# strawberrylady99/mythril

Measured on AMD Instinct MI355X. Metric: candidate assignments evaluated/sec (node) + time-to-first-model vs z3, higher is better.
Workload: dtype u32

## Files before the change

### mythril_amd/csrc/jit_asm.cpp

```cpp
#include <algorithm>
#include <array>
#include <cstdio>
#include <cstring>
#include <functional>
#include <map>
#include <set>
#include <sstream>
#include <string>
#include <vector>

#include "jit.hpp"

namespace mg {

namespace {

struct AsmFail {
  std::string why;
};
[[noreturn]] void fail(const std::string& w) { throw AsmFail{w}; }

inline uint32_t Lw(uint32_t w) { return (w + 31) / 32; }
inline uint32_t topmask(uint32_t w) { return (w & 31) ? ((1u << (w & 31)) - 1u) : 0xFFFFFFFFu; }
inline uint32_t gsalt(uint32_t c, uint32_t j) { return c * 0x9E3779B9u + j * 0x85EBCA6Bu + 0x27D4EB2Fu; }
// ... 31 lines not shown
  snprintf(b, sizeof b, "0x%x", x);
  return b;
}
bool inl(uint32_t x) {
  const int32_t s = (int32_t)x;
  return s >= -16 && s <= 64;
}
std::string imm(uint32_t x) { return inl(x) ? std::to_string((int32_t)x) : hexs(x); }
std::string V(uint32_t r) { return "v" + std::to_string(r); }
std::string S(uint32_t r) { return "s" + std::to_string(r); }
std::string SP(uint32_t r) { return "s[" + std::to_string(r) + ":" + std::to_string(r + 1) + "]"; }
std::string VP(uint32_t r) { return "v[" + std::to_string(r) + ":" + std::to_string(r + 1) + "]"; }

constexpr int kV0 = 12;
constexpr int kS0 = 44, kS1 = 100;

class Emitter {
 public:
  std::ostringstream o;
  int64_t pos = 0;
  std::map<int, int64_t> vw;
  int nlab = 0;
  std::vector<int> vref = std::vector<int>(256, 0);
  std::vector<uint32_t> vgen = std::vector<uint32_t>(256, 0);
  uint32_t gen_ctr = 0;
  static bool check_on() {
    static const bool on = [] {
      const char* g = getenv("MYTHGPU_JIT_ASM_CHECK");
      return g && g[0] == '1';
    }();
// ... 738 lines not shown
        E.valu("v_add3_u32 " + VL(vj) + ", " + VL(vj) + ", " + VL(ve) + ", " + (inl(base) ? imm(base) : "s41"), {41});
        E.valu("v_lshlrev_b32_e32 " + VL(vj) + ", 2, " + VL(vj));
        drop(vi);
        drop(ve);
        pend.push_back({vt, vj});
        if (pend.size() >= stage_batch()) flush();
      }
    }
    flush();
    E.ctl("s_waitcnt lgkmcnt(0)");
    E.ctl("s_barrier");
  }

  Emitter& e() { return E; }

  int cond = 0;
  static constexpr int kCondPairs = 8;
  void sreserve() {
    while (E.sfree() < kCondPairs && E.on_spressure && E.on_spressure()) {
    }
  }
  struct CondScope {
    Gen& g;
    explicit CondScope(Gen& g_) : g(g_) {
      if (!g.cond) g.sreserve();
      g.cond++;
    }
    ~CondScope() { g.cond--; }
  };
  std::map<uint32_t, Limb> litcache;
// ... 395 lines not shown
      const uint32_t e = cnt == 1 ? first : miss;
      const std::string op = cnt == 1 ? "v_cmp_eq_u32" : "v_cmp_ne_u32";
      if (inl(e)) {
        E.valu(op + "_e64 " + SP(m.s) + ", " + imm(e) + ", " + VL(idx), {}, {m.s, m.s + 1});
      } else {
        E.valu(op + "_e32 vcc, " + hexs(e) + ", " + VL(idx), {}, {kVCC, kVCC + 1});
        E.salu("s_mov_b64 " + SP(m.s) + ", vcc", {m.s, m.s + 1});
      }
      mcache_put(ck, m);
      return true;
    }
    uint32_t bits = 0;
    for (uint32_t e = 0; e < n; e++)
      if (S[e]) bits |= 1u << e;
    const Limb t = fresh();
    E.salu("s_mov_b32 s41, " + hexs(bits), {41});
    E.valu("v_bfe_u32 " + VL(t) + ", s41, " + VL(idx) + ", 1", {41});
    E.valu("v_cmp_ne_u32_e64 " + SP(m.s) + ", 0, " + VL(t), {}, {m.s, m.s + 1});
    drop(t);
    mcache_put(ck, m);
    return true;
  }
  bool dict_eq(const std::vector<std::pair<Limb, Limb>>& prs, Mask& m) {
    if (no_dict_eq() || dlimb.empty()) return false;
    bool haveA = false, haveB = false;
    DLimb A, B;
    std::vector<std::pair<uint32_t, uint32_t>> lits;
    std::vector<std::pair<uint32_t, uint32_t>> regs;
    auto same_src = [](const DLimb& x, const DLimb& y) {
      return x.off == y.off && x.n == y.n && x.Lc == y.Lc && x.idx == y.idx && x.idx.g == y.idx.g;
    };
    for (const auto& pr : prs) {
// ... 912 lines not shown
    const Limb d = into ? *into : fresh(), t = fresh();
    const uint32_t salt = gsalt(c, j);
    if (no_kfold()) {
      E.valu("v_xor_b32_e32 " + VL(d) + ", " + imm(salt) + ", v4");
      E.valu("v_xor_b32_sdwa " + VL(d) + ", " + VL(d) + ", " + VL(d) +
             " dst_sel:DWORD dst_unused:UNUSED_PAD src0_sel:DWORD src1_sel:WORD_1");
    } else {
      E.valu("v_xor_b32_e32 " + VL(d) + ", " + imm(salt ^ (salt >> 16)) + ", v4");
    }
    E.valu("v_mul_u32_u24_e32 " + VL(d) + ", 0x9e3779, " + VL(d));
    E.valu("v_lshrrev_b32_e32 " + VL(t) + ", 15, " + VL(d));
    E.valu("v_xad_u32 " + VL(d) + ", " + VL(t) + ", " + VL(d) + ", v5");
    drop(t);
    return d;
  }
  void gwsel(uint32_t c, int s) {
    E.salu("s_xor_b32 " + S(s) + ", s36, " + hexs(gsalt(c, 0xFFFEu)), {s});
    E.salu("s_mul_i32 " + S(s) + ", " + S(s) + ", 0x9e3779b1", {s});
    E.salu("s_add_u32 " + S(s) + ", " + S(s) + ", s37", {s});
  }
  std::vector<Limb> uniform_limbs(uint32_t c, uint32_t Lc, uint32_t bits, const std::vector<Limb>* tgt = nullptr) {
    const uint32_t n = std::min(Lc, (bits + 31) / 32);
    if (tgt) {
      std::vector<Limb> r(*tgt);
      for (uint32_t j = 0; j < n; j++) {
        if (j < 2) {
          grnd(c, j, &r[j]);
        } else {
          const uint32_t s = (7u * j + 3u) % 31u + 1u;
          E.valu("v_alignbit_b32 " + VL(r[j]) + ", " + VL(r[j - 1]) + ", " + VL(r[j - 2]) + ", " + std::to_string(s));
// ... 48 lines not shown
  }
  std::vector<Limb> add_lit(const uint32_t* lo, uint32_t Lc, const std::vector<Limb>& off, uint32_t k) {
    std::vector<Limb> a(k), b(k);
    for (uint32_t j = 0; j < k; j++) {
      a[j] = Lit(lo[j]);
      b[j] = j < off.size() ? off[j] : Lit(0);
    }
    std::vector<Limb> r = add_chain(a, b, k, false);
    r.resize(Lc);
    for (uint32_t j = k; j < Lc; j++) r[j] = Lit(lo[j]);
    return r;
  }
  Limb mulhi_lit(const Limb& x, uint32_t c) {
    if (x.lit()) return Lit((uint32_t)(((uint64_t)x.v * c) >> 32));
    const Limb d = fresh();
    if (inl(c)) {
      E.valu("v_mul_hi_u32 " + VL(d) + ", " + VL(x) + ", " + imm(c));
    } else {
      E.salu("s_mov_b32 s41, " + hexs(c), {41});
      E.valu("v_mul_hi_u32 " + VL(d) + ", " + VL(x) + ", s41", {41});
    }
    return d;
  }

  std::vector<Limb> dict(uint32_t off, uint32_t n, uint32_t w, const Limb& idx, const std::vector<Limb>* tgt = nullptr,
                         uint32_t upto = 64) {
    const uint32_t Lc = Lw(w), Lu = std::min(Lc, upto);
    std::vector<Limb> r(Lc, Lit(0));
    auto dst = [&](uint32_t j) { return tgt ? (*tgt)[j] : fresh(); };
    if (w <= 32 && n && (uint64_t)n * w <= 32) {
      uint32_t pack = 0;
      const uint32_t m = w == 32 ? 0xFFFFFFFFu : ((1u << w) - 1u);
      for (uint32_t e2 = 0; e2 < n; e2++) pack |= (G[off + e2] & m) << (e2 * w);
      const Limb sh = fresh(), d = dst(0);
      E.valu("v_mul_u32_u24_e32 " + VL(sh) + ", " + imm(w) + ", " + VL(idx));
      E.salu("s_mov_b32 s41, " + hexs(pack), {41});
      E.valu("v_bfe_u32 " + VL(d) + ", s41, " + VL(sh) + ", " + std::to_string(w), {41});
      drop(sh);
      r[0] = d;
      return r;
    }
    if (n <= 4 && !lds_base.count(off)) {
      std::vector<Mask> ms;
      for (uint32_t e2 = 0; e2 + 1 < n; e2++) {
        Mask m;
        m.k = 2;
        m.s = E.salloc();
        E.valu("v_cmp_ne_u32_e64 " + SP(m.s) + ", " + std::to_string(e2) + ", " + VL(idx), {}, {m.s, m.s + 1});
        ms.push_back(m);
      }
      std::map<std::vector<uint32_t>, Limb> memo;
      std::function<Limb(uint32_t, uint32_t)> chain = [&](uint32_t j, uint32_t e) -> Limb {
// ... 168 lines not shown
    E.valu("v_lshrrev_b32_e32 " + VL(e2) + ", 16, " + VL(e2));
    return e2;
  }

  void put(const std::vector<Limb>& out, std::vector<Limb>& r) {
    for (size_t j = 0; j < out.size(); j++) {
      const Limb x = j < r.size() ? r[j] : Lit(0);
      if (x == out[j]) continue;
      E.valu("v_mov_b32_e32 " + VL(out[j]) + ", " + src(x));
      if (j < r.size()) drop(r[j]);
    }
    for (size_t j = out.size(); j < r.size(); j++) drop(r[j]);
    r.clear();
  }

  void delta(const std::vector<Limb>& out, uint32_t c, uint32_t pdelta, int ws, const Limb* hknown) {
    CondScope cs_(*this);
    const std::string skip = E.newlab();
    E.salu("s_and_b32 s40, " + S(ws) + ", 0xffff", {40});
    E.salu("s_cmp_lt_u32 s40, " + imm(pdelta));
    E.ctl("s_cbranch_scc0 " + skip);
    Limb h = hknown ? *hknown : grnd(c, 0xFFFFu);
    if (hknown) E.retain(h);
    const Limb mag = fresh(), neg = fresh();
    Mask sb;
    sb.k = 2;
    sb.s = E.salloc();
    E.valu("v_and_b32_e32 " + VL(mag) + ", 1, " + VL(h));
    E.valu("v_add_u32_e32 " + VL(mag) + ", 1, " + VL(mag));
    E.valu("v_bfe_u32 " + VL(neg) + ", " + VL(h) + ", 1, 1");
    E.valu("v_cmp_ne_u32_e64 " + SP(sb.s) + ", 0, " + VL(neg), {}, {sb.s, sb.s + 1});
    E.valu("v_sub_u32_e32 " + VL(neg) + ", 0, " + VL(mag));
    E.valu("v_cndmask_b32_e64 " + VL(mag) + ", " + VL(mag) + ", " + VL(neg) + ", " + SP(sb.s), {sb.s, sb.s + 1});
    drop(neg);
    const uint32_t Lc = (uint32_t)out.size();
// ... 38 lines not shown
        bad = mnot(z);
        E.srelease(z);
      }
      if (span) {
        Mask ge;
        ge.k = 2;
        ge.s = E.salloc();
        Limb d0 = out[0];
        if (G[r]) {
          d0 = fresh();
          E.valu("v_subrev_u32_e32 " + VL(d0) + ", " + imm(G[r]) + ", " + VL(out[0]));
        }
        if (inl(span)) {
          E.valu("v_cmp_le_u32_e64 " + SP(ge.s) + ", " + imm(span) + ", " + VL(d0), {}, {ge.s, ge.s + 1});
        } else {
          E.salu("s_mov_b32 s41, " + hexs(span), {41});
          E.valu("v_cmp_le_u32_e64 " + SP(ge.s) + ", s41, " + VL(d0), {41}, {ge.s, ge.s + 1});
        }
        if (G[r]) drop(d0);
        const Mask b2 = mop("or", bad, ge);
        E.srelease(ge);
        E.srelease(bad);
        bad = b2;
      }
      if (bad.k == 1 && !bad.ones) return;
      Limb c0;
      if (span) {
        c0 = mulhi_lit(out[0], span);
        if (G[r]) E.valu("v_add_u32_e32 " + VL(c0) + ", " + imm(G[r]) + ", " + VL(c0));
      }
      mask_to_vcc(bad);
      if (span) {
// ... 18 lines not shown
    for (uint32_t j = 1; j < Lc; j++) hz.push_back({dif[j], Lit(0)});
    if (!hz.empty()) {
      const Mask z = eq_mask(hz);
      const Mask nz = mnot(z);
      const Mask b2 = mop("or", bad, nz);
      E.srelease(z);
      E.srelease(nz);
      E.srelease(bad);
      bad = b2;
    }
    if (span) {
      Mask ge;
      ge.k = 2;
      ge.s = E.salloc();
      const Limb d0 = vreg(dif[0]);
      E.salu("s_mov_b32 s41, " + hexs(span), {41});
      E.valu("v_cmp_le_u32_e64 " + SP(ge.s) + ", s41, " + VL(d0), {41}, {ge.s, ge.s + 1});
      drop(d0);
      const Mask b2 = mop("or", bad, ge);
      E.srelease(ge);
      E.srelease(bad);
      bad = b2;
    }
    for (auto& d : dif) drop(d);
    std::vector<Limb> offv(1);
    offv[0] = span ? mulhi_lit(out[0], span) : out[0];
    if (!span) E.retain(out[0]);
    std::vector<Limb> cl = add_lit(&G[r], Lc, offv, k);
    drop(offv[0]);
    mask_to_vcc(bad);
    for (uint32_t j = 0; j < Lc; j++) {
      Limb t = cl[j], tmp;
// ... 28 lines not shown
        r[j] = Lit(x);
        continue;
      }
      const Limb a = and_lit(r[j], ~m);
      drop(r[j]);
      r[j] = a;
      if (v) {
        const Limb d = fresh();
        E.valu("v_or_b32_e32 " + VL(d) + ", " + imm(v) + ", " + VL(a));
        drop(a);
        r[j] = d;
      }
    }
  }

  std::vector<Limb> gen_value(uint32_t c, uint64_t want = ~0ull) {
    const GenSpec sp = specs.at(c);
    const uint32_t fix = sp.kind >> 8, kind = sp.kind & 0xFFu;
    const uint32_t width = P.coord_width.at(c), Lc = Lw(width);
    std::vector<Limb> r;
    switch (kind) {
      case MG_GEN_MIXED: {
        uint64_t wl = want & lowmask(Lc);
        if (fix)
          for (uint32_t j = 0; j < Lc; j++)
            if (G[fix - 1 + j] == 0xFFFFFFFFu) wl &= ~(1ull << j);
        const uint32_t Lg = (sp.p[6] || no_gen_want()) ? Lc : (wl ? 64u - (uint32_t)__builtin_clzll(wl) : 0u);
        if (Lg == 0) {
          r.assign(Lc, Lit(0));
          if (fix) fixbits(r, fix, false);
          return r;
        }
        CondScope cs_(*this);
        std::vector<Limb> out(Lg);
        if (lds_pairs() && sp.p[1] && (sp.p[2] >> 16) && lds_base.count(sp.p[0])) {
          for (uint32_t j = 0; j < Lg; j += 2) {
            if (j + 1 < Lg) {
              const uint32_t rr = E.valloc2();
              out[j] = Limb{LR, rr, E.vgen[rr]};
              out[j + 1] = Limb{LR, rr + 1, E.vgen[rr + 1]};
            } else {
              out[j] = fresh();
            }
          }
        } else {
          for (auto& x : out) x = fresh();
        }
        const uint32_t pc = sp.p[3] != MG_NONE ? (sp.p[2] & 0xFFFFu) : 0u;
        const uint32_t pd = sp.p[1] ? (sp.p[2] >> 16) : 0u;
        const uint32_t ps = sp.p[4] & 0xFFFFu;
        const uint32_t small_bits = std::min(width, sp.p[4] >> 16);
        const bool narrow = width <= MG_GEN_NARROW_BITS;
        const int ws = E.salloc();
        gwsel(c, ws);
        const std::string end = E.newlab();
        auto uni = [&](uint32_t bitsn) {
          std::vector<Limb> u;
          if (narrow) {
            const Limb h = grnd(c, 0xFFFFu);
            u.assign(Lc, Lit(0));
            const uint32_t m = bitsn >= 32 ? 0xFFFFFFFFu : ((1u << bitsn) - 1u);
            u[0] = and_lit(h, m & 0xFFFFu);
            drop(h);
          } else {
            u = uniform_limbs(c, Lg, bitsn, &out);
          }
          put(out, u);
        };
        std::string next;
        bool any = false;
        auto branch = [&](uint32_t T) {
          if (any) {
            E.ctl("s_branch " + end);
            E.label(next);
          }
          any = true;
          next = E.newlab();
          if (T < 65536u) {
            E.salu("s_cmp_lt_u32 " + S(ws) + ", " + hexs(T << 16));
            E.ctl("s_cbranch_scc0 " + next);
          }
        };
        note("mixed:key");
        if (pc) {
          branch(pc);
          note("mixed:copy");
          std::vector<Limb> s;
          auto it = cval.find(sp.p[3]);
          if (debug_live() && it != cval.end())
            fprintf(stderr, "asm copy source %u of %u: def %d need %llx\n", sp.p[3], c, (int)val[it->second].def,
                    (unsigned long long)need[it->second]);
          if (it != cval.end() && val[it->second].def &&
              (need[it->second] & lowmask(L(it->second))) == lowmask(L(it->second))) {
            s = val[it->second].l;
            for (auto& x : s) E.retain(x);
          } else {
            s = gen_value(sp.p[3], lowmask(Lg));
          }
          uint64_t zero = 0;
          for (uint32_t j = 0; j < Lc && !sp.p[5]; j++)
            if (j < s.size() && s[j].lit() && s[j].v == 0) zero |= 1ull << j;
          put(out, s);
          if (sp.p[5]) delta(out, c, sp.p[5], ws, nullptr);
          finish(out, width, sp.p[6], zero);
        }
        if (pd) {
          branch(pc + pd);
          note("mixed:dict");
          const Limb h = grnd(c, 0xFFFFu);
          const Limb ix = dict_index(h, sp.p[1]);
          std::vector<Limb> dv = dict(sp.p[0], sp.p[1], width, ix, &out, Lg);
          drop(ix);
          uint64_t zero = 0;
          for (uint32_t j = 0; j < Lc && !sp.p[5]; j++)
            if (j < dv.size() && dv[j].lit() && dv[j].v == 0) zero |= 1ull << j;
          put(out, dv);
          if (sp.p[5]) delta(out, c, sp.p[5], ws, &h);
          drop(h);
          finish(out, width, sp.p[6], zero);
        }
        auto zeros = [&](uint32_t bitsn) {
          uint64_t z = 0;
          for (uint32_t j = 0; j < Lc; j++)
            if ((narrow && j > 0) || 32 * j >= bitsn) z |= 1ull << j;
          return z;
        };
        if (ps) {
          branch(pc + pd + ps);
          note("mixed:small");
          uni(small_bits);
          finish(out, width, sp.p[6], zeros(small_bits));
        }
        if (any) {
          E.ctl("s_branch " + end);
          E.label(next);
        }
        note("mixed:uniform");
        uni(width);
        finish(out, width, sp.p[6], zeros(width));
        E.label(end);
        note("mixed:join");
        Mask wsm;
        wsm.k = 2;
        wsm.s = ws;
        E.srelease(wsm);
        r.assign(Lc, Lit(0));
        for (uint32_t j = 0; j < Lg; j++) r[j] = out[j];
        if (fix) {
          const uint32_t f = fix - 1;
          for (uint32_t j = 0; j < Lc; j++) {
            const uint32_t m = G[f + j], v = G[f + Lc + j];
            if (!m) continue;
            if (!r[j].reg() || m == 0xFFFFFFFFu) {
              drop(r[j]);
              r[j] = Lit(v);
              continue;
            }
            E.valu("v_and_b32_e32 " + VL(r[j]) + ", " + imm(~m) + ", " + VL(r[j]));
            if (v) E.valu("v_or_b32_e32 " + VL(r[j]) + ", " + imm(v) + ", " + VL(r[j]));
          }
        }
        return r;
      }
      case MG_GEN_DICT: {
        const Limb h = grnd(c, 0xFFFFu);
        const Limb ix = dict_index(h, sp.p[1]);
        drop(h);
        r = dict(sp.p[0], sp.p[1], width, ix);
        std::vector<Limb> rd = r;
// ... 29 lines not shown
        break;
      }
      case MG_GEN_ALIGNED: {
        const Limb rr = grnd(c, 0);
        Limb m;
        if (sp.p[2]) {
          m = mulhi_lit(rr, sp.p[2]);
          drop(rr);
        } else {
          m = rr;
        }
        const int32_t sh = (int32_t)sp.p[1];
        const uint32_t k = reach_limbs(&G[sp.p[0]], Lc, sp.p[2] ? sp.p[2] - 1u : 0xFFFFFFFFull, (uint32_t)sh);
        if (aligned_mad() && k == 2 && Lc >= 2 && sh > 0 && sh <= 6 && m.reg()) {
          const uint32_t rp = E.valloc2();
          E.salu("s_mov_b32 s40, " + hexs(G[sp.p[0]]), {40});
          E.salu("s_mov_b32 s41, " + hexs(G[sp.p[0] + 1]), {41});
          Mask cm;
          cm.k = 2;
          cm.s = E.salloc();
          E.valu("v_mad_u64_u32 v[" + std::to_string(rp) + ":" + std::to_string(rp + 1) + "], " + SP(cm.s) + ", " + VL(m) +
                     ", " + std::to_string(1 << sh) + ", s[40:41]",
                 {40, 41}, {cm.s, cm.s + 1});
          E.srelease(cm);
          drop(m);
          r.assign(Lc, Lit(0));
          r[0] = Limb{LR, rp, E.vgen[rp]};
          r[1] = Limb{LR, rp + 1, E.vgen[rp + 1]};
          for (uint32_t j = 2; j < Lc; j++) r[j] = Lit(G[sp.p[0] + j]);
          break;
        }
        std::vector<Limb> mw(Lc, Lit(0));
        for (uint32_t j = 0; j < Lc; j++) {
          const int32_t bit0 = (int32_t)(j * 32) - sh;
          if (bit0 <= -32 || bit0 >= 32) continue;
          const Limb d = fresh();
          if (bit0 < 0) E.valu("v_lshlrev_b32_e32 " + VL(d) + ", " + std::to_string(-bit0) + ", " + VL(m));
          else if (bit0 > 0) E.valu("v_lshrrev_b32_e32 " + VL(d) + ", " + std::to_string(bit0) + ", " + VL(m));
// ... 166 lines not shown
  }
  Mask mask_new() {
    Mask m;
    m.k = 2;
    m.s = E.salloc();
    return m;
  }
  void vsel(const Limb& d, const Limb& f, const Limb& t, const Mask& m) {
    E.valu("v_cndmask_b32_e64 " + VL(d) + ", " + VL(f) + ", " + VL(t) + ", " + SP(m.s), {m.s, m.s + 1});
  }
  Mask vcmp(const char* op, const Limb& a, uint32_t k) {
    Mask m = mask_new();
    if (inl(k)) {
      E.valu(std::string("v_cmp_") + op + "_u32_e64 " + SP(m.s) + ", " + VL(a) + ", " + imm(k), {}, {m.s, m.s + 1});
    } else {
      E.salu("s_mov_b32 s41, " + hexs(k), {41});
      E.valu(std::string("v_cmp_") + op + "_u32_e64 " + SP(m.s) + ", " + VL(a) + ", s41", {41}, {m.s, m.s + 1});
    }
    return m;
  }

  Limb bitlen(const std::vector<Limb>& x) {
    const Limb bl = fresh();
    E.valu("v_mov_b32_e32 " + VL(bl) + ", 0");
    for (uint32_t j = 0; j < x.size(); j++) {
      const Limb l = x[j];
      if (l.k == LU || (l.lit() && l.v == 0)) continue;
      if (l.lit()) {
        E.valu("v_mov_b32_e32 " + VL(bl) + ", " + imm(32 * j + 32 - (uint32_t)__builtin_clz(l.v)));
        continue;
      }
      const Limb t = fresh();
// ... 1450 lines not shown
          E.srelease(h);
        }
        set(d, cur);
        break;
      }
      case K_ASSERT: {
        litcache_clear();
        const Mask m = mask_of(in.a);
        if (m.k == 1) {
          if (!m.ones) E.salu("s_mov_b64 s[38:39], 0", {38, 39});
        } else {
          E.salu("s_and_b64 s[38:39], s[38:39], " + SP(m.s), {38, 39});
        }
        bool later = false;
        for (size_t q = k + 1; q < code.size() && !later; q++) later = code[q].op == K_ASSERT;
        if (!gen_kernel && !eval_kernel && later) {
          E.salu("s_or_b64 s[40:41], s[38:39], s[42:43]", {40, 41});
          E.ctl("s_cbranch_scc0 " + next);
        }
        break;
      }
      case K_WATCH:
        if (eval_kernel) {
          CondScope cs_(*this);
          const uint32_t Lw_ = Lw(P.vwidth[in.a]);
          E.salu("s_cmp_eq_u64 s[12:13], 0");
          const std::string skip = E.newlab();
          E.ctl("s_cbranch_scc1 " + skip);
          E.salu("s_mov_b64 exec, s[24:25]");
          for (uint32_t j = 0; j < Lw_; j++) {
            const Limb x = vreg(limb(in.a, j));
// ... 655 lines not shown
      if (st != std::string::npos) res.replace(st, 18, hexs(spill_stride()));
    }
    return res;
  }

  uint32_t eval_lds_bytes() const {
    return (glds ? 4u * glds_slots() * 256u : 0u) + (spill_on ? (solo ? 1u : 4u) * spill_stride() * 256u : 0u);
  }

  int labels = 0;
  std::string kernel(const std::string& name) {
    E = Emitter();
    E.nlab = labels;
    E.vsoft = vsoft;
    census.clear();
    E.vfirst = kV0 + (int)pool.size();
    E.vhigh = E.vfirst;
    val.assign(P.vwidth.size(), Val{});
    cval.clear();
    auto& o = E.o;
    o << "  .text\n  .globl " << name << "\n  .p2align 8\n  .type " << name << ",@function\n" << name << ":\n";
    E.ctl("s_load_dwordx2 s[4:5], s[0:1], 0x0");
    E.ctl("s_load_dwordx8 s[8:15], s[0:1], 0x8");
    if (gen_kernel) {
      E.ctl("s_load_dwordx2 s[16:17], s[0:1], 0x28");
      E.ctl("s_load_dword s19, s[0:1], 0x30");
    } else {
      E.ctl("s_load_dwordx4 s[16:19], s[0:1], 0x28");
    }
    E.valu("v_and_b32_e32 v1, 63, v0");
    E.valu("v_mov_b32_e32 v6, 0");
// ... 20 lines not shown
    E.salu("s_lshl_b32 s28, s19, 2", {28});
    E.salu("s_mov_b64 s[30:31], -1", {30, 31});
    E.salu("s_mov_b64 s[32:33], 0", {32, 33});
    for (const auto& kv : pool) E.valu("v_mov_b32_e32 " + V((uint32_t)kv.second) + ", " + imm(kv.first));
    E.valu("v_xor_b32_e32 v2, s12, v1", {12});
    E.valu("v_mov_b32_e32 v3, s13", {13});
    vfmix(2, 3);
    E.salu("s_and_b32 s12, s22, 0xffffffc0", {12});
    E.salu("s_mov_b32 s13, s23", {13});
    E.salu("s_and_b32 s40, s22, 63", {40});
    E.salu("s_cmp_lg_u32 s40, 0");
    E.salu("s_cselect_b64 s[12:13], s[12:13], -1", {12, 13});
    E.salu("s_and_b32 s40, s8, 63", {40});
    E.salu("s_cmp_lg_u32 s40, 0");
    E.salu("s_cselect_b64 s[10:11], s[20:21], -1", {10, 11});
    E.salu("s_movk_i32 s7, 0x40", {7});
    const std::string loop = E.newlab(), exit_ = E.newlab(), next = E.newlab(), cont = E.newlab();
    E.label(loop);
    E.salu("s_sub_u32 s40, s26, s24", {40});
    E.salu("s_subb_u32 s40, s27, s25", {40});
    E.ctl("s_cbranch_scc0 " + exit_);
    E.salu("s_lshl_b64 s[34:35], s[26:27], 6", {34, 35});
    E.salu("s_add_u32 s34, s34, s20", {34});
    E.salu("s_addc_u32 s35, s35, s21", {35});
    if (!gen_kernel) {
      const std::string noearly = E.newlab();
      E.salu("s_cmp_eq_u32 s29, 0");
      E.ctl("s_cbranch_scc1 " + noearly);
      {
        const std::string sys = E.newlab(), got = E.newlab();
        E.salu("s_and_b32 s40, s18, 2", {40});
        E.ctl("s_cbranch_scc1 " + sys);
        E.mem("global_load_dwordx2 v[8:9], v6, s[16:17] sc1", {16, 17});
        E.ctl("s_branch " + got);
        E.label(sys);
        E.mem("global_load_dwordx2 v[8:9], v6, s[16:17] sc0 sc1", {16, 17});
        E.label(got);
      }
      E.ctl("s_waitcnt vmcnt(0)");
      E.valu("v_readfirstlane_b32 s40, v8", {}, {40});
      E.valu("v_readfirstlane_b32 s41, v9", {}, {41});
      E.salu("s_sub_u32 s40, s34, s40", {40});
      E.salu("s_subb_u32 s40, s35, s41", {40});
      E.ctl("s_cbranch_scc0 " + exit_);
      E.label(noearly);
    }
    if (salu_group_key()) {
      E.salu("s_lshr_b64 s[36:37], s[34:35], 6", {36, 37});
      E.salu("s_xor_b64 s[36:37], s[36:37], s[14:15]", {36, 37});
      sfmix(36);
    } else {
      const std::string have = E.newlab();
      E.salu("s_cmp_lt_u32 s7, 64");
      E.ctl("s_cbranch_scc1 " + have);
      E.valu("v_mul_u32_u24_e32 v10, s28, v1", {28});
      E.valu("v_lshrrev_b64 v[8:9], 6, s[20:21]", {20, 21});
      E.valu("v_add_co_u32_e32 v10, vcc, s26, v10", {26}, {kVCC, kVCC + 1});
      E.valu("v_mov_b32_e32 v11, s27", {27});
      E.valu("v_addc_co_u32_e32 v11, vcc, 0, v11, vcc", {kVCC, kVCC + 1}, {kVCC, kVCC + 1});
      E.valu("v_add_co_u32_e32 v10, vcc, v8, v10", {}, {kVCC, kVCC + 1});
      E.valu("v_addc_co_u32_e32 v11, vcc, v9, v11, vcc", {kVCC, kVCC + 1}, {kVCC, kVCC + 1});
      E.valu("v_xor_b32_e32 v10, s14, v10", {14});
      E.valu("v_xor_b32_e32 v11, s15, v11", {15});
      vfmix(10, 11);
      E.salu("s_mov_b32 s7, 0", {7});
      E.label(have);
      E.valu("v_readlane_b32 s36, v10, s7", {7}, {36});
      E.valu("v_readlane_b32 s37, v11, s7", {7}, {37});
      E.salu("s_add_u32 s7, s7, 1", {7});
    }
    E.valu("v_xor_b32_e32 v4, s36, v2", {36});
    if (!no_kfold())
      E.valu("v_xor_b32_sdwa v4, v4, v4 dst_sel:DWORD dst_unused:UNUSED_PAD src0_sel:DWORD src1_sel:WORD_1");
    E.valu("v_xor_b32_e32 v5, s37, v3", {37});
    E.salu("s_mov_b64 s[38:39], -1", {38, 39});
    {
      static const std::array<int, 3> pad = [] {
        const char* g = getenv("MYTHGPU_JIT_ASM_DIAG_PAD");
        int a = 0, b = 0, c = 0;
        if (g) sscanf(g, "%d,%d,%d", &a, &b, &c);
        return std::array<int, 3>{std::max(0, std::min(a, 200)), std::max(0, std::min(b, 200)), std::max(0, std::min(c, 200))};
      }();
      for (int q = 0; q < pad[0]; q++) E.salu("s_mov_b32 s40, s40", {40});
      for (int q = 0; q < pad[1]; q++) E.valu("v_mov_b32_e32 v7, 0");
// ... 80 lines not shown
        E.valu("v_readfirstlane_b32 s50, v8", {}, {50});
        E.valu("v_readfirstlane_b32 s51, v9", {}, {51});
        E.valu("v_mov_b32_e32 v8, s46", {46});
        E.valu("v_mov_b32_e32 v9, s47", {47});
        E.mem("global_atomic_umin_x2 v6, v[8:9], s[50:51] sc1", {50, 51});
        E.salu("s_add_u32 s49, s49, 1", {49});
        E.salu("s_cmp_lt_u32 s49, s48");
        E.ctl("s_cbranch_scc1 " + ploop);
        E.label(pdone);
      }
      E.salu("s_mov_b64 exec, -1");
    }
    E.label(cont);
    E.salu("s_add_u32 s26, s26, s28", {26});
    E.salu("s_addc_u32 s27, s27, 0", {27});
    E.ctl("s_branch " + loop);
    E.label(exit_);
    if (!gen_kernel) {
      const std::string nobest = E.newlab(), end = E.newlab();
      E.salu("s_cmp_eq_u64 s[30:31], -1");
      E.ctl("s_cbranch_scc1 " + nobest);
      if (exit_skip()) {
        E.salu("s_mov_b64 exec, 1");
        E.mem("global_load_dwordx2 v[8:9], v6, s[16:17]", {16, 17});
        E.ctl("s_waitcnt vmcnt(0)");
        E.valu("v_readfirstlane_b32 s46, v8", {}, {46});
        E.valu("v_readfirstlane_b32 s47, v9", {}, {47});
        E.salu("s_mov_b64 exec, -1");
        E.salu("s_sub_u32 s44, s30, s46", {44});
        E.salu("s_subb_u32 s44, s31, s47", {44});
        E.ctl("s_cbranch_scc0 " + nobest);
// ... 6 lines not shown
      E.label(nobest);
      E.salu("s_cmp_eq_u64 s[32:33], 0");
      E.ctl("s_cbranch_scc1 " + end);
      E.salu("s_and_b32 s40, s2, 15", {40});
      E.salu("s_add_u32 s40, s40, 1", {40});
      E.salu("s_lshl_b32 s40, s40, 7", {40});
      E.salu("s_add_u32 s44, s16, s40", {44});
      E.salu("s_addc_u32 s45, s17, 0", {45});
      E.salu("s_mov_b64 exec, 1");
      E.valu("v_mov_b32_e32 v8, s32", {32});
      E.valu("v_mov_b32_e32 v9, s33", {33});
      E.mem("global_atomic_add_x2 v6, v[8:9], s[44:45]", {44, 45});
      E.label(end);
    }
    E.ctl("s_endpgm");
    mcache_note();
    static const int diag_vgprs = [] {
      const char* g = getenv("MYTHGPU_JIT_ASM_DIAG_VGPRS");
      return g ? std::max(0, std::min(256, atoi(g))) : 0;
    }();
    const int nv = std::max({E.vhigh, kV0, diag_vgprs}), ns = std::max(E.shigh, 56);
    const int accum = (nv + 3) / 4 * 4;
    o << "  .section .rodata,\"a\",@progbits\n  .p2align 6, 0x0\n  .amdhsa_kernel " << name << "\n"
      << "    .amdhsa_group_segment_fixed_size " << lds_words * 4 << "\n    .amdhsa_private_segment_fixed_size 0\n"
      << "    .amdhsa_kernarg_size " << (gen_kernel ? 52 : 56) << "\n"
      << "    .amdhsa_user_sgpr_count 2\n    .amdhsa_user_sgpr_kernarg_segment_ptr 1\n"
      << "    .amdhsa_system_sgpr_workgroup_id_x 1\n    .amdhsa_system_vgpr_workitem_id 0\n"
      << "    .amdhsa_next_free_vgpr " << nv << "\n    .amdhsa_next_free_sgpr " << ns << "\n"
      << "    .amdhsa_accum_offset " << accum << "\n    .amdhsa_reserve_vcc 1\n"
      << "    .amdhsa_float_denorm_mode_32 3\n    .amdhsa_float_denorm_mode_16_64 3\n"
// ... 197 lines not shown
      out = o.str();
      return MG_OK;
    }
    g.analyse();
    g.gen_kernel = false;
    g.caches = false;
    std::string ks;
    int v0;
    try {
      ks = g.kernel("mgj_search");
      v0 = g.meta_vgpr["mgj_search"];
      if (getenv("MYTHGPU_JIT_ASM_VREPORT")) fprintf(stderr, "mythgpu asm: pass-1 VGPRs %d\n", v0);
    } catch (const AsmFail&) {
      v0 = 256;
      g.census.clear();
    }
    g.caches = true;
    g.vsoft = occupancy_step(v0);
    if (Gen::sgkey_env() >= 0) {
      g.sgkey = Gen::sgkey_env() == 1;
    } else if (!ks.empty()) {
      size_t sa = 0, va = 0;
      std::istringstream in(ks);
      for (std::string ln; std::getline(in, ln);) {
        if (ln.rfind("  v_", 0) == 0) va++;
        else if (ln.rfind("  s_", 0) == 0 && ln.rfind("  s_waitcnt", 0) && ln.rfind("  s_nop", 0) &&
                 ln.rfind("  s_branch", 0) && ln.rfind("  s_cbranch", 0) && ln.rfind("  s_endpgm", 0))
          sa++;
      }
      g.sgkey = va && (double)sa < kSgkeyRatio * (double)va;
    }
    {
      std::vector<std::pair<uint32_t, uint32_t>> by;
      static const uint32_t pool_min = [] {
        const char* g = getenv("MYTHGPU_JIT_ASM_POOL_MIN");
        return g ? (uint32_t)std::max(1, atoi(g)) : 2u;
      }();
      if (!getenv("MYTHGPU_JIT_ASM_NOPOOL"))
        for (const auto& kv : g.census)
          if (kv.second >= pool_min) by.push_back({kv.second, kv.first});
      std::sort(by.begin(), by.end(), [](const auto& a, const auto& b) { return a.first > b.first; });
      const int room = std::max(0, std::min(96, g.vsoft) - v0);
      for (size_t i = 0; i < by.size() && (int)i < room; i++) g.pool[by[i].second] = kV0 + (int)i;
      g.labels = 0;
      ks = g.kernel("mgj_search");
    }
    o << ks;
    const bool with_gen = (kernels & JIT_GEN) != 0;
    if (with_gen) {
      g.gen_kernel = true;
      o << g.kernel("mgj_gen");
    }
    o << metadata(g.meta_vgpr, g.meta_sgpr, with_gen, g.meta_lds);
    out = o.str();
    return MG_OK;
  } catch (const AsmFail& f) {
    err = f.why;
// ... 9 lines not shown
```

Measured before the change: 276.8 billion.

## Pool scalar literals, rotate loop test, cold assert stubs, power-of-two mulhi shifts

Adds several independent codegen tweaks to the JIT assembler. Frequently used 32/64-bit literals are counted and hoisted into reserved SGPRs (s6/s7) set once before the loop. The loop-bound check is rotated to the bottom, asserts with SGPR masks branch to out-of-line stubs, power-of-two mulhi becomes a shift, and mixed generators can write into borrowed target registers. A per-class precomputed bit table that replaces per-iteration scalar hashing is added but left disabled by default. The extra live SGPRs/VGPRs and new code paths add register pressure and correctness risk.

```diff
diff --git a/mythril_amd/csrc/jit_asm.cpp b/mythril_amd/csrc/jit_asm.cpp
--- a/mythril_amd/csrc/jit_asm.cpp
+++ b/mythril_amd/csrc/jit_asm.cpp
@@ -69,6 +69,10 @@
 
 constexpr int kV0 = 12;
 constexpr int kS0 = 44, kS1 = 100;
+
+constexpr bool kClassTableDefault = false;
+constexpr bool kSlitDefault = true;
+constexpr bool kSmallCutsDefault = true;
 
 class Emitter {
  public:
@@ -837,6 +841,33 @@
 
   Emitter& e() { return E; }
 
+  std::map<uint32_t, uint32_t> scensus;
+  std::map<uint64_t, uint32_t> scensus64;
+  std::map<uint32_t, int> spool;
+  std::map<uint64_t, int> spool64;
+  static bool no_slit() {
+    static const bool on = [] {
+      const char* g = getenv("MYTHGPU_JIT_ASM_NO_SLIT");
+      return g ? g[0] != '0' : !kSlitDefault;
+    }();
+    return on;
+  }
+  int slit(uint32_t v) {
+    scensus[v] += cond ? 1u : 4u;
+    auto it = spool.find(v);
+    if (it != spool.end()) return it->second;
+    E.salu("s_mov_b32 s41, " + hexs(v), {41});
+    return 41;
+  }
+  int slit64(uint32_t lo, uint32_t hi) {
+    const uint64_t v = ((uint64_t)hi << 32) | lo;
+    scensus64[v] += cond ? 1u : 4u;
+    auto it = spool64.find(v);
+    if (it != spool64.end()) return it->second;
+    E.salu("s_mov_b32 s40, " + hexs(lo), {40});
+    E.salu("s_mov_b32 s41, " + hexs(hi), {41});
+    return 40;
+  }
   int cond = 0;
   static constexpr int kCondPairs = 8;
   void sreserve() {
@@ -1262,8 +1293,8 @@
     for (uint32_t e = 0; e < n; e++)
       if (S[e]) bits |= 1u << e;
     const Limb t = fresh();
-    E.salu("s_mov_b32 s41, " + hexs(bits), {41});
-    E.valu("v_bfe_u32 " + VL(t) + ", s41, " + VL(idx) + ", 1", {41});
+    const int sb = slit(bits);
+    E.valu("v_bfe_u32 " + VL(t) + ", s" + std::to_string(sb) + ", " + VL(idx) + ", 1", {sb});
     E.valu("v_cmp_ne_u32_e64 " + SP(m.s) + ", 0, " + VL(t), {}, {m.s, m.s + 1});
     drop(t);
     mcache_put(ck, m);
@@ -2206,6 +2237,112 @@
     drop(t);
     return d;
   }
+  struct CSlot {
+    int word = 0;
+    int bit = 0;
+    int nthr = 0;
+  };
+  struct MixClasses {
+    uint32_t n = 0;
+    uint32_t k[4] = {0, 0, 0, 0};
+    uint32_t T[4] = {0, 0, 0, 0};
+    bool flag = false;
+    uint32_t bits() const { return n - 1 + (flag ? 1u : 0u); }
+  };
+  static MixClasses mix_classes(const GenSpec& sp) {
+    MixClasses m;
+    const uint32_t pc = sp.p[3] != MG_NONE ? (sp.p[2] & 0xFFFFu) : 0u;
+    const uint32_t pd = sp.p[1] ? (sp.p[2] >> 16) : 0u;
+    const uint32_t ps = sp.p[4] & 0xFFFFu;
+    uint32_t cum = 0;
+    const uint32_t part[3] = {pc, pd, ps};
+    for (uint32_t q = 0; q < 3 && cum < 65536u; q++) {
+      if (!part[q]) continue;
+      cum += part[q];
+      m.k[m.n] = q;
+      m.T[m.n++] = std::min(cum, 65536u);
+      if (q < 2 && sp.p[5]) m.flag = true;
+    }
+    if (cum < 65536u) {
+      m.k[m.n] = 3;
+      m.T[m.n++] = 65536u;
+    }
+    return m;
+  }
+  static bool no_class_table() {
+    static const bool on = [] {
+      const char* g = getenv("MYTHGPU_JIT_ASM_NO_CLASS_TABLE");
+      return g ? g[0] != '0' : !kClassTableDefault;
+    }();
+    return on;
+  }
+  static bool no_small_cuts() {
+    static const bool on = [] {
+      const char* g = getenv("MYTHGPU_JIT_ASM_NO_SMALL_CUTS");
+      return g ? g[0] != '0' : !kSmallCutsDefault;
+    }();
+    return on;
+  }
+  std::vector<std::pair<std::string, std::string>> assert_stubs;
+  std::string assert_next;
+  std::vector<uint32_t> ctab_seen;
+  std::map<uint32_t, CSlot> ctab;
+  std::vector<std::vector<uint32_t>> ctab_word;
+  int ctab_v0() const { return kV0 + (int)pool.size(); }
+  static int ctab_sgpr(int w) { return w == 0 ? 1 : 6; }
+  void ctab_assign() {
+    ctab.clear();
+    ctab_word.clear();
+    if (no_class_table()) return;
+    uint32_t used = 32;
+    for (uint32_t c : ctab_seen) {
+      const uint32_t b = mix_classes(specs.at(c)).bits();
+      if (!b) continue;
+      if (used + b > 32) {
+        if (ctab_word.size() == 2) break;
+        ctab_word.emplace_back();
+        used = 0;
+      }
+      CSlot s;
+      s.word = ctab_sgpr((int)ctab_word.size() - 1);
+      s.bit = (int)used;
+      s.nthr = (int)mix_classes(specs.at(c)).n - 1;
+      ctab[c] = s;
+      ctab_word.back().push_back(c);
+      used += b;
+    }
+  }
+  void ctab_fill() {
+    if (ctab_word.empty()) return;
+    const Limb t = fresh(), t2 = fresh();
+    E.salu("s_mov_b32 s40, 0x9e3779b1", {40});
+    for (size_t w = 0; w < ctab_word.size(); w++) {
+      const std::string W = V((uint32_t)(ctab_v0() + (int)w));
+      E.valu("v_mov_b32_e32 " + W + ", 0");
+      auto shift_in = [&]() {
+        E.valu("v_addc_co_u32_e32 " + W + ", vcc, " + W + ", " + W + ", vcc", {kVCC, kVCC + 1}, {kVCC, kVCC + 1});
+      };
+      for (size_t q = ctab_word[w].size(); q-- > 0;) {
+        const uint32_t c = ctab_word[w][q];
+        const GenSpec& sp = specs.at(c);
+        const MixClasses m = mix_classes(sp);
+        E.valu("v_xor_b32_e32 " + VL(t) + ", " + imm(gsalt(c, 0xFFFEu)) + ", v10");
+        E.valu("v_mul_lo_u32 " + VL(t) + ", " + VL(t) + ", s40", {40});
+        E.valu("v_add_u32_e32 " + VL(t) + ", v11, " + VL(t));
+        if (m.flag) {
+          E.valu("v_and_b32_e32 " + VL(t2) + ", 0xffff, " + VL(t));
+          E.valu("v_cmp_gt_u32_e32 vcc, " + imm(sp.p[5]) + ", " + VL(t2), {}, {kVCC, kVCC + 1});
+          shift_in();
+        }
+        for (uint32_t j = m.n - 1; j-- > 0;) {
+          E.valu("v_cmp_gt_u32_e32 vcc, " + imm(m.T[j] << 16) + ", " + VL(t), {}, {kVCC, kVCC + 1});
+          shift_in();
+        }
+      }
+    }
+    drop(t);
+    drop(t2);
+  }
   void gwsel(uint32_t c, int s) {
     E.salu("s_xor_b32 " + S(s) + ", s36, " + hexs(gsalt(c, 0xFFFEu)), {s});
     E.salu("s_mul_i32 " + S(s) + ", " + S(s) + ", 0x9e3779b1", {s});
@@ -2284,11 +2421,13 @@
   Limb mulhi_lit(const Limb& x, uint32_t c) {
     if (x.lit()) return Lit((uint32_t)(((uint64_t)x.v * c) >> 32));
     const Limb d = fresh();
-    if (inl(c)) {
+    if (!no_small_cuts() && c > 1 && !(c & (c - 1))) {
+      E.valu("v_lshrrev_b32_e32 " + VL(d) + ", " + std::to_string(32 - __builtin_ctz(c)) + ", " + VL(x));
+    } else if (inl(c)) {
       E.valu("v_mul_hi_u32 " + VL(d) + ", " + VL(x) + ", " + imm(c));
     } else {
-      E.salu("s_mov_b32 s41, " + hexs(c), {41});
-      E.valu("v_mul_hi_u32 " + VL(d) + ", " + VL(x) + ", s41", {41});
+      const int sc = slit(c);
+      E.valu("v_mul_hi_u32 " + VL(d) + ", " + VL(x) + ", " + S(sc), {sc});
     }
     return d;
   }
@@ -2304,8 +2443,8 @@
       for (uint32_t e2 = 0; e2 < n; e2++) pack |= (G[off + e2] & m) << (e2 * w);
       const Limb sh = fresh(), d = dst(0);
       E.valu("v_mul_u32_u24_e32 " + VL(sh) + ", " + imm(w) + ", " + VL(idx));
-      E.salu("s_mov_b32 s41, " + hexs(pack), {41});
-      E.valu("v_bfe_u32 " + VL(d) + ", s41, " + VL(sh) + ", " + std::to_string(w), {41});
+      const int sp_ = slit(pack);
+      E.valu("v_bfe_u32 " + VL(d) + ", " + S(sp_) + ", " + VL(sh) + ", " + std::to_string(w), {sp_});
       drop(sh);
       r[0] = d;
       return r;
@@ -2504,11 +2643,16 @@
     r.clear();
   }
 
-  void delta(const std::vector<Limb>& out, uint32_t c, uint32_t pdelta, int ws, const Limb* hknown) {
+  void delta(const std::vector<Limb>& out, uint32_t c, uint32_t pdelta, int ws, const Limb* hknown,
+             const CSlot* cs = nullptr) {
     CondScope cs_(*this);
     const std::string skip = E.newlab();
-    E.salu("s_and_b32 s40, " + S(ws) + ", 0xffff", {40});
-    E.salu("s_cmp_lt_u32 s40, " + imm(pdelta));
+    if (cs) {
+      E.salu("s_bitcmp1_b32 " + S(cs->word) + ", " + std::to_string(cs->bit + cs->nthr));
+    } else {
+      E.salu("s_and_b32 s40, " + S(ws) + ", 0xffff", {40});
+      E.salu("s_cmp_lt_u32 s40, " + imm(pdelta));
+    }
     E.ctl("s_cbranch_scc0 " + skip);
     Limb h = hknown ? *hknown : grnd(c, 0xFFFFu);
     if (hknown) E.retain(h);
@@ -2577,8 +2721,8 @@
         if (inl(span)) {
           E.valu("v_cmp_le_u32_e64 " + SP(ge.s) + ", " + imm(span) + ", " + VL(d0), {}, {ge.s, ge.s + 1});
         } else {
-          E.salu("s_mov_b32 s41, " + hexs(span), {41});
-          E.valu("v_cmp_le_u32_e64 " + SP(ge.s) + ", s41, " + VL(d0), {41}, {ge.s, ge.s + 1});
+          const int ss = slit(span);
+          E.valu("v_cmp_le_u32_e64 " + SP(ge.s) + ", " + S(ss) + ", " + VL(d0), {ss}, {ge.s, ge.s + 1});
         }
         if (G[r]) drop(d0);
         const Mask b2 = mop("or", bad, ge);
@@ -2627,8 +2771,8 @@
       ge.k = 2;
       ge.s = E.salloc();
       const Limb d0 = vreg(dif[0]);
-      E.salu("s_mov_b32 s41, " + hexs(span), {41});
-      E.valu("v_cmp_le_u32_e64 " + SP(ge.s) + ", s41, " + VL(d0), {41}, {ge.s, ge.s + 1});
+      const int ss = slit(span);
+      E.valu("v_cmp_le_u32_e64 " + SP(ge.s) + ", " + S(ss) + ", " + VL(d0), {ss}, {ge.s, ge.s + 1});
       drop(d0);
       const Mask b2 = mop("or", bad, ge);
       E.srelease(ge);
@@ -2687,7 +2831,7 @@
     }
   }
 
-  std::vector<Limb> gen_value(uint32_t c, uint64_t want = ~0ull) {
+  std::vector<Limb> gen_value(uint32_t c, uint64_t want = ~0ull, const std::vector<Limb>* tgt = nullptr) {
     const GenSpec sp = specs.at(c);
     const uint32_t fix = sp.kind >> 8, kind = sp.kind & 0xFFu;
     const uint32_t width = P.coord_width.at(c), Lc = Lw(width);
@@ -2706,7 +2850,16 @@
         }
         CondScope cs_(*this);
         std::vector<Limb> out(Lg);
-        if (lds_pairs() && sp.p[1] && (sp.p[2] >> 16) && lds_base.count(sp.p[0])) {
+        const bool pairs = lds_pairs() && sp.p[1] && (sp.p[2] >> 16) && lds_base.count(sp.p[0]);
+        bool borrowed = tgt && tgt->size() >= Lg;
+        for (uint32_t j = 0; borrowed && j < Lg; j++) {
+          borrowed = (*tgt)[j].reg();
+          if (borrowed && pairs && !(j & 1) && j + 1 < Lg)
+            borrowed = !((*tgt)[j].v & 1) && (*tgt)[j + 1].reg() && (*tgt)[j + 1].v == (*tgt)[j].v + 1;
+        }
+        if (borrowed) {
+          for (uint32_t j = 0; j < Lg; j++) out[j] = (*tgt)[j];
+        } else if (pairs) {
           for (uint32_t j = 0; j < Lg; j += 2) {
             if (j + 1 < Lg) {
               const uint32_t rr = E.valloc2();
@@ -2724,8 +2877,16 @@
         const uint32_t ps = sp.p[4] & 0xFFFFu;
         const uint32_t small_bits = std::min(width, sp.p[4] >> 16);
         const bool narrow = width <= MG_GEN_NARROW_BITS;
-        const int ws = E.salloc();
-        gwsel(c, ws);
+        if (std::find(ctab_seen.begin(), ctab_seen.end(), c) == ctab_seen.end()) ctab_seen.push_back(c);
+        const MixClasses mc = mix_classes(sp);
+        const auto slot = ctab.find(c);
+        const bool tabled = slot != ctab.end() || (!no_class_table() && mc.bits() == 0);
+        const CSlot* cs = slot != ctab.end() ? &slot->second : nullptr;
+        int ws = -1;
+        if (!tabled) {
+          ws = E.salloc();
+          gwsel(c, ws);
+        }
         const std::string end = E.newlab();
         auto uni = [&](uint32_t bitsn) {
           std::vector<Limb> u;
@@ -2755,8 +2916,7 @@
           }
         };
         note("mixed:key");
-        if (pc) {
-          branch(pc);
+        auto body_copy = [&]() {
           note("mixed:copy");
           std::vector<Limb> s;
           auto it = cval.find(sp.p[3]);
@@ -2768,17 +2928,16 @@
             s = val[it->second].l;
             for (auto& x : s) E.retain(x);
           } else {
-            s = gen_value(sp.p[3], lowmask(Lg));
+            s = gen_value(sp.p[3], lowmask(Lg), no_small_cuts() ? nullptr : &out);
           }
           uint64_t zero = 0;
           for (uint32_t j = 0; j < Lc && !sp.p[5]; j++)
             if (j < s.size() && s[j].lit() && s[j].v == 0) zero |= 1ull << j;
           put(out, s);
-          if (sp.p[5]) delta(out, c, sp.p[5], ws, nullptr);
+          if (sp.p[5]) delta(out, c, sp.p[5], ws, nullptr, cs);
           finish(out, width, sp.p[6], zero);
-        }
-        if (pd) {
-          branch(pc + pd);
+        };
+        auto body_dict = [&]() {
           note("mixed:dict");
           const Limb h = grnd(c, 0xFFFFu);
           const Limb ix = dict_index(h, sp.p[1]);
@@ -2788,35 +2947,86 @@
           for (uint32_t j = 0; j < Lc && !sp.p[5]; j++)
             if (j < dv.size() && dv[j].lit() && dv[j].v == 0) zero |= 1ull << j;
           put(out, dv);
-          if (sp.p[5]) delta(out, c, sp.p[5], ws, &h);
+          if (sp.p[5]) delta(out, c, sp.p[5], ws, &h, cs);
           drop(h);
           finish(out, width, sp.p[6], zero);
-        }
+        };
         auto zeros = [&](uint32_t bitsn) {
           uint64_t z = 0;
           for (uint32_t j = 0; j < Lc; j++)
             if ((narrow && j > 0) || 32 * j >= bitsn) z |= 1ull << j;
           return z;
         };
-        if (ps) {
-          branch(pc + pd + ps);
+        auto body_small = [&]() {
           note("mixed:small");
           uni(small_bits);
           finish(out, width, sp.p[6], zeros(small_bits));
-        }
-        if (any) {
-          E.ctl("s_branch " + end);
-          E.label(next);
-        }
-        note("mixed:uniform");
-        uni(width);
-        finish(out, width, sp.p[6], zeros(width));
+        };
+        auto body_uniform = [&]() {
+          note("mixed:uniform");
+          uni(width);
+          finish(out, width, sp.p[6], zeros(width));
+        };
+        if (tabled) {
+          uint32_t cost[5][5] = {}, cut[5][5] = {};
+          for (uint32_t len = 2; len <= mc.n; len++)
+            for (uint32_t a = 0; a + len <= mc.n; a++) {
+              const uint32_t b = a + len, span = mc.T[b - 1] - (a ? mc.T[a - 1] : 0u);
+              cost[a][b] = ~0u;
+              for (uint32_t s = a + 1; s < b; s++)
+                if (cost[a][s] + cost[s][b] < cost[a][b]) {
+                  cost[a][b] = cost[a][s] + cost[s][b];
+                  cut[a][b] = s;
+                }
+              cost[a][b] += span;
+            }
+          std::function<void(uint32_t, uint32_t)> tree = [&](uint32_t a, uint32_t b) {
+            if (b - a == 1) {
+              switch (mc.k[a]) {
+                case 0: body_copy(); break;
+                case 1: body_dict(); break;
+                case 2: body_small(); break;
+                default: body_uniform(); break;
+              }
+              return;
+            }
+            const uint32_t s = cut[a][b];
+            const std::string right = E.newlab();
+            E.salu("s_bitcmp1_b32 " + S(cs->word) + ", " + std::to_string(cs->bit + (int)s - 1));
+            E.ctl("s_cbranch_scc0 " + right);
+            tree(a, s);
+            E.ctl("s_branch " + end);
+            E.label(right);
+            tree(s, b);
+          };
+          tree(0, mc.n);
+        } else {
+          if (pc) {
+            branch(pc);
+            body_copy();
+          }
+          if (pd) {
+            branch(pc + pd);
+            body_dict();
+          }
+          if (ps) {
+            branch(pc + pd + ps);
+            body_small();
+          }
+          if (any) {
+            E.ctl("s_branch " + end);
+            E.label(next);
+          }
+          body_uniform();
+        }
         E.label(end);
         note("mixed:join");
-        Mask wsm;
-        wsm.k = 2;
-        wsm.s = ws;
-        E.srelease(wsm);
+        if (ws >= 0) {
+          Mask wsm;
+          wsm.k = 2;
+          wsm.s = ws;
+          E.srelease(wsm);
+        }
         r.assign(Lc, Lit(0));
         for (uint32_t j = 0; j < Lg; j++) r[j] = out[j];
         if (fix) {
@@ -2825,7 +3035,7 @@
             const uint32_t m = G[f + j], v = G[f + Lc + j];
             if (!m) continue;
             if (!r[j].reg() || m == 0xFFFFFFFFu) {
-              drop(r[j]);
+              if (!borrowed) drop(r[j]);
               r[j] = Lit(v);
               continue;
             }
@@ -2885,14 +3095,13 @@
         const uint32_t k = reach_limbs(&G[sp.p[0]], Lc, sp.p[2] ? sp.p[2] - 1u : 0xFFFFFFFFull, (uint32_t)sh);
         if (aligned_mad() && k == 2 && Lc >= 2 && sh > 0 && sh <= 6 && m.reg()) {
           const uint32_t rp = E.valloc2();
-          E.salu("s_mov_b32 s40, " + hexs(G[sp.p[0]]), {40});
-          E.salu("s_mov_b32 s41, " + hexs(G[sp.p[0] + 1]), {41});
+          const int sb = slit64(G[sp.p[0]], G[sp.p[0] + 1]);
           Mask cm;
           cm.k = 2;
           cm.s = E.salloc();
           E.valu("v_mad_u64_u32 v[" + std::to_string(rp) + ":" + std::to_string(rp + 1) + "], " + SP(cm.s) + ", " + VL(m) +
-                     ", " + std::to_string(1 << sh) + ", s[40:41]",
-                 {40, 41}, {cm.s, cm.s + 1});
+                     ", " + std::to_string(1 << sh) + ", " + SP(sb),
+                 {sb, sb + 1}, {cm.s, cm.s + 1});
           E.srelease(cm);
           drop(m);
           r.assign(Lc, Lit(0));
@@ -3089,8 +3298,8 @@
     if (inl(k)) {
       E.valu(std::string("v_cmp_") + op + "_u32_e64 " + SP(m.s) + ", " + VL(a) + ", " + imm(k), {}, {m.s, m.s + 1});
     } else {
-      E.salu("s_mov_b32 s41, " + hexs(k), {41});
-      E.valu(std::string("v_cmp_") + op + "_u32_e64 " + SP(m.s) + ", " + VL(a) + ", s41", {41}, {m.s, m.s + 1});
+      const int sk = slit(k);
+      E.valu(std::string("v_cmp_") + op + "_u32_e64 " + SP(m.s) + ", " + VL(a) + ", " + S(sk), {sk}, {m.s, m.s + 1});
     }
     return m;
   }
@@ -4571,7 +4780,13 @@
         }
         bool later = false;
         for (size_t q = k + 1; q < code.size() && !later; q++) later = code[q].op == K_ASSERT;
-        if (!gen_kernel && !eval_kernel && later) {
+        if (!gen_kernel && !eval_kernel && later && m.k == 2 && !no_small_cuts()) {
+          const std::string stub = E.newlab(), back = E.newlab();
+          E.ctl("s_cbranch_scc0 " + stub);
+          E.o << back << ":\n";
+          assert_stubs.push_back({stub, back});
+          assert_next = next;
+        } else if (!gen_kernel && !eval_kernel && later) {
           E.salu("s_or_b64 s[40:41], s[38:39], s[42:43]", {40, 41});
           E.ctl("s_cbranch_scc0 " + next);
         }
@@ -5257,7 +5472,10 @@
     E.nlab = labels;
     E.vsoft = vsoft;
     census.clear();
-    E.vfirst = kV0 + (int)pool.size();
+    scensus.clear();
+    scensus64.clear();
+    E.vfirst = ctab_v0() + (int)ctab_word.size();
+    assert_stubs.clear();
     E.vhigh = E.vfirst;
     val.assign(P.vwidth.size(), Val{});
     cval.clear();
@@ -5308,12 +5526,26 @@
     E.salu("s_and_b32 s40, s8, 63", {40});
     E.salu("s_cmp_lg_u32 s40, 0");
     E.salu("s_cselect_b64 s[10:11], s[20:21], -1", {10, 11});
-    E.salu("s_movk_i32 s7, 0x40", {7});
+    const int kl = no_slit() ? 7 : 0;
+    const std::string KL = S((uint32_t)kl);
+    E.salu("s_movk_i32 " + KL + ", 0x40", {kl});
+    for (const auto& kv : spool) E.salu("s_mov_b32 " + S(kv.second) + ", " + hexs(kv.first), {kv.second});
+    for (const auto& kv : spool64) {
+      E.salu("s_mov_b32 " + S(kv.second) + ", " + hexs((uint32_t)kv.first), {kv.second});
+      E.salu("s_mov_b32 " + S(kv.second + 1) + ", " + hexs((uint32_t)(kv.first >> 32)), {kv.second + 1});
+    }
     const std::string loop = E.newlab(), exit_ = E.newlab(), next = E.newlab(), cont = E.newlab();
+    if (!no_small_cuts()) {
+      E.salu("s_sub_u32 s40, s26, s24", {40});
+      E.salu("s_subb_u32 s40, s27, s25", {40});
+      E.ctl("s_cbranch_scc0 " + exit_);
+    }
     E.label(loop);
-    E.salu("s_sub_u32 s40, s26, s24", {40});
-    E.salu("s_subb_u32 s40, s27, s25", {40});
-    E.ctl("s_cbranch_scc0 " + exit_);
+    if (no_small_cuts()) {
+      E.salu("s_sub_u32 s40, s26, s24", {40});
+      E.salu("s_subb_u32 s40, s27, s25", {40});
+      E.ctl("s_cbranch_scc0 " + exit_);
+    }
     E.salu("s_lshl_b64 s[34:35], s[26:27], 6", {34, 35});
     E.salu("s_add_u32 s34, s34, s20", {34});
     E.salu("s_addc_u32 s35, s35, s21", {35});
@@ -5339,13 +5571,9 @@
       E.ctl("s_cbranch_scc0 " + exit_);
       E.label(noearly);
     }
-    if (salu_group_key()) {
-      E.salu("s_lshr_b64 s[36:37], s[34:35], 6", {36, 37});
-      E.salu("s_xor_b64 s[36:37], s[36:37], s[14:15]", {36, 37});
-      sfmix(36);
-    } else {
+    if (!salu_group_key() || !ctab_word.empty()) {
       const std::string have = E.newlab();
-      E.salu("s_cmp_lt_u32 s7, 64");
+      E.salu("s_cmp_lt_u32 " + KL + ", 64");
       E.ctl("s_cbranch_scc1 " + have);
       E.valu("v_mul_u32_u24_e32 v10, s28, v1", {28});
       E.valu("v_lshrrev_b64 v[8:9], 6, s[20:21]", {20, 21});
@@ -5357,11 +5585,22 @@
       E.valu("v_xor_b32_e32 v10, s14, v10", {14});
       E.valu("v_xor_b32_e32 v11, s15, v11", {15});
       vfmix(10, 11);
-      E.salu("s_mov_b32 s7, 0", {7});
+      ctab_fill();
+      E.salu("s_mov_b32 " + KL + ", 0", {kl});
       E.label(have);
-      E.valu("v_readlane_b32 s36, v10, s7", {7}, {36});
-      E.valu("v_readlane_b32 s37, v11, s7", {7}, {37});
-      E.salu("s_add_u32 s7, s7, 1", {7});
+      if (!salu_group_key()) {
+        E.valu("v_readlane_b32 s36, v10, " + KL, {kl}, {36});
+        E.valu("v_readlane_b32 s37, v11, " + KL, {kl}, {37});
+      }
+      for (size_t w = 0; w < ctab_word.size(); w++)
+        E.valu("v_readlane_b32 " + S(ctab_sgpr((int)w)) + ", " + V((uint32_t)(ctab_v0() + (int)w)) + ", " + KL, {kl},
+               {ctab_sgpr((int)w)});
+      E.salu("s_add_u32 " + KL + ", " + KL + ", 1", {kl});
+    }
+    if (salu_group_key()) {
+      E.salu("s_lshr_b64 s[36:37], s[34:35], 6", {36, 37});
+      E.salu("s_xor_b64 s[36:37], s[36:37], s[14:15]", {36, 37});
+      sfmix(36);
     }
     E.valu("v_xor_b32_e32 v4, s36, v2", {36});
     if (!no_kfold())
@@ -5472,7 +5711,13 @@
     E.label(cont);
     E.salu("s_add_u32 s26, s26, s28", {26});
     E.salu("s_addc_u32 s27, s27, 0", {27});
-    E.ctl("s_branch " + loop);
+    if (!no_small_cuts()) {
+      E.salu("s_sub_u32 s40, s26, s24", {40});
+      E.salu("s_subb_u32 s40, s27, s25", {40});
+      E.ctl("s_cbranch_scc1 " + loop);
+    } else {
+      E.ctl("s_branch " + loop);
+    }
     E.label(exit_);
     if (!gen_kernel) {
       const std::string nobest = E.newlab(), end = E.newlab();
@@ -5509,6 +5754,12 @@
       E.label(end);
     }
     E.ctl("s_endpgm");
+    for (const auto& st : assert_stubs) {
+      E.o << st.first << ":\n";
+      E.salu("s_cmp_lg_u32 s29, 0");
+      E.ctl("s_cbranch_scc1 " + assert_next);
+      E.ctl("s_branch " + st.second);
+    }
     mcache_note();
     static const int diag_vgprs = [] {
       const char* g = getenv("MYTHGPU_JIT_ASM_DIAG_VGPRS");
@@ -5736,6 +5987,9 @@
     } catch (const AsmFail&) {
       v0 = 256;
       g.census.clear();
+      g.scensus.clear();
+      g.scensus64.clear();
+      g.ctab_seen.clear();
     }
     g.caches = true;
     g.vsoft = occupancy_step(v0);
@@ -5762,7 +6016,29 @@
         for (const auto& kv : g.census)
           if (kv.second >= pool_min) by.push_back({kv.second, kv.first});
       std::sort(by.begin(), by.end(), [](const auto& a, const auto& b) { return a.first > b.first; });
-      const int room = std::max(0, std::min(96, g.vsoft) - v0);
+      g.ctab_assign();
+      if (v0 + (int)g.ctab_word.size() > g.vsoft) {
+        g.ctab.clear();
+        g.ctab_word.clear();
+      }
+      if (!Gen::no_slit()) {
+        std::vector<std::pair<uint32_t, uint32_t>> s32;
+        for (const auto& kv : g.scensus)
+          if (kv.second >= 5) s32.push_back({kv.second, kv.first});
+        std::sort(s32.begin(), s32.end(), [](const auto& a, const auto& b) { return a > b; });
+        std::pair<uint32_t, uint64_t> s64{0, 0};
+        for (const auto& kv : g.scensus64)
+          if (kv.second >= 5 && kv.second > s64.first) s64 = {kv.second, kv.first};
+        const bool s6free = g.ctab_word.size() < 2;
+        const uint32_t gain32 = (s32.size() > 0 ? s32[0].first : 0u) + (s6free && s32.size() > 1 ? s32[1].first : 0u);
+        if (s6free && 2 * s64.first > gain32) {
+          g.spool64[s64.second] = 6;
+        } else {
+          if (s32.size() > 0) g.spool[s32[0].second] = 7;
+          if (s6free && s32.size() > 1) g.spool[s32[1].second] = 6;
+        }
+      }
+      const int room = std::max(0, std::min(96, g.vsoft) - v0 - (int)g.ctab_word.size());
       for (size_t i = 0; i < by.size() && (int)i < room; i++) g.pool[by[i].second] = kV0 + (int)i;
       g.labels = 0;
       ks = g.kernel("mgj_search");
```

After: 284.5 billion, median of 4. +2.8%, better.
